# AdeeshKolluru/AdsorbDiff

Measured on AMD Instinct MI355X. Metric: sampled adsorbate sites/sec (50 denoise steps, ~200-atom slabs), higher is better.
Workload: dtype f32 (f16x3-split MFMA, fp32 accumulate; ADF_GEMM=f32 selects exact f32)

## Files before the change

adsorbdiff_amd/csrc/api.hip:

```cpp
#include <stdarg.h>
#include <stdlib.h>
#include <string.h>

#include <new>

#include "common.h"

static thread_local char g_err[512] = "";

void adf_set_error(const char* fmt, ...) {
    va_list ap;
    va_start(ap, fmt);
    vsnprintf(g_err, sizeof(g_err), fmt, ap);
    va_end(ap);
}

extern "C" const char* adf_last_error(void) { return g_err; }
extern "C" const char* adf_version(void) { return "adsorbdiff_hip 0.5.0 (gfx950)"; }

void adf_prof_begin(adf_painn* h, int cat, hipStream_t s) {
    if (!h->prof_on) return;
    if (h->prof_used + 2 > h->prof_ev->size()) {
        for (int i = 0; i < 512; ++i) {
            hipEvent_t e;
// ... 119 lines not shown
        if (st == ADF_OK) st = dev_alloc(&h->w16_scratch, 1);
        if (st == ADF_OK) st = dev_alloc(&h->wfrag_arena, h->w16_bytes);
        {
            const char* ef = getenv("ADF_FUSED_MLP");
            h->fused_mlp = ef ? atoi(ef) : 0;
            if (h->fused_mlp < 0 || h->fused_mlp > 2) h->fused_mlp = 0;
        }
        const char* e = getenv("ADF_GEMM");
        h->gemm_f32 = e && strcmp(e, "f32") == 0;
        const char* el = getenv("ADF_LIFT");
        h->lift_on = !(el && strcmp(el, "0") == 0);
        const char* e2 = getenv("ADF_MSG");
        h->msg_f32 = e2 ? strcmp(e2, "f32") == 0 : h->gemm_f32;
        const char* er = getenv("ADF_ROW_MAXIMA");
        h->rmx = (er && atoi(er) == 0) ? 0 : 1;
    }
    if (st == ADF_OK) st = dev_alloc(&h->kcount, 8);
    if (st == ADF_OK && hipMemset(h->kcount, 0, 8 * sizeof(unsigned long long)) != hipSuccess) st = ADF_EHIP;
    if (st != ADF_OK) { adf_painn_destroy(h); return st; }
    *out = h;
    return ADF_OK;
}

static void inc_free(adf_painn* h) {
    for (int l = 0; l <= ADF_MAX_LAYERS; ++l) {
        if (h->incX[l]) (void)hipFree(h->incX[l]);
        if (h->incV[l]) (void)hipFree(h->incV[l]);
        if (l < ADF_MAX_LAYERS && h->incR[l]) (void)hipFree(h->incR[l]);
        h->incX[l] = h->incV[l] = nullptr;
        if (l < ADF_MAX_LAYERS) h->incR[l] = nullptr;
// ... 295 lines not shown
    if (nbr_src) ADF_HIP_CHECK(hipMemcpyAsync(nbr_src, h->nbr_src, sizeof(int32_t) * N * K, hipMemcpyDeviceToDevice, s));
    if (nbr_shift)
        hipLaunchKernelGGL(adf_export_shift_kernel, dim3((unsigned)((N * K + 255) / 256)), dim3(256), 0, s, h->nbr_shift,
                           nbr_shift, (long long)(N * K), h->last_reps[0], h->last_reps[1], h->last_reps[2]);
    if (edge_src || edge_dst || edge_dist || edge_vec)
        hipLaunchKernelGGL(adf_export_edges_kernel, dim3((unsigned)((N + 3) / 4)), dim3(256), 0, s, h->nptr, h->e_src,
                           h->e_geom, (int)N, edge_src, edge_dst, edge_dist, edge_vec, (long long)edge_capacity);
    ADF_HIP_CHECK(hipGetLastError());
    int32_t e = 0;
    ADF_HIP_CHECK(hipMemcpyAsync(&e, h->nptr + N, sizeof(int32_t), hipMemcpyDeviceToHost, s));
    ADF_HIP_CHECK(hipStreamSynchronize(s));
    if (num_edges) *num_edges = e;
    return ADF_OK;
}

static int32_t zero_pad_rows(adf_painn* h, int N, hipStream_t s) {
    const size_t row = (size_t)5 * h->hp.hidden_channels;
    ADF_HIP_CHECK(hipMemsetAsync(h->rec + (size_t)N * row, 0, sizeof(float) * row, s));
    return ADF_OK;
}

static bool use_fused_mlp(const adf_painn* h, int rows) {
    if (h->hp.hidden_channels != 512 || h->gemm_f32 || h->fused_mlp == 0) return false;
    if (h->fused_mlp == 1) return true;
    return rows >= 2 * 64 * h->num_cus;
}

static int32_t make_records(adf_painn* h, int l, int n, const float* x, const float* vec, bool vec_is_zero, float* rec,
                            const int32_t* row_map, hipStream_t s) {
    const int H = h->hp.hidden_channels;
    const adf_layer_weights& w = h->layer[l];
    if (n <= 0) return ADF_OK;
    adf_prof_begin(h, ADF_PROF_NODE, s);
    const bool lift = h->lift_on && !h->gemm_f32;
    static int emit = -1;
    if (emit < 0) { const char* e = getenv("ADF_LIFT_EMIT"); emit = (e && atoi(e) == 0) ? 0 : 1; }
    const bool em = lift && emit;
    ADF_TRY(adf_nodewise_layernorm(x, w.ln_w, w.ln_b, h->y, n, H, s, em ? h->mag_a : nullptr, h->rows_dev));
    if (use_fused_mlp(h, n) && (em || !lift)) {
        adf_epi ep = {};
        ep.vec_in = vec; ep.rec = rec ? rec : h->rec; ep.H = H; ep.vec_is_zero = vec_is_zero ? 1 : 0;
        ep.row_map = row_map; ep.m_dev = h->rows_dev; ep.lift_y = lift ? 1 : 0;
        ep.rec_rows = row_map ? (long long)h->inc_capN : (long long)n;
        ADF_TRY(adf_launch_mlp16(h->y, nullptr, H, em ? h->mag_a : nullptr, w.xp0_16.frag, &w.xp0_16, w.xp0_b, w.xp2_16.frag, &w.xp2_16, n,
                                 H, 1, &ep, s));
        adf_prof_end(h, s);
        return ADF_OK;
    }
    ADF_TRY(adf_linear(h, h->y, H, w.xp0_w, &w.xp0_16, w.xp0_b, h->cat, H, n, H, H, 1, s, em ? h->mag_a : nullptr,
                       em ? h->mag_b : nullptr));
    if (h->gemm_f32) {
        if (row_map) { adf_set_error("internal: mapped records need the f16x3 path"); return ADF_EINVAL; }
        ADF_TRY(adf_launch_gemm(h->cat, H, w.xp2_w, H, w.xp2_b, h->xh, 3 * H, n, 3 * H, H, 0, s));
        ADF_TRY(adf_pack_records(h, n, h->xh, vec, vec_is_zero, s, rec));
    } else {
        adf_epi ep = {};
        ep.vec_in = vec; ep.rec = rec ? rec : h->rec; ep.H = H; ep.vec_is_zero = vec_is_zero ? 1 : 0;
        ep.row_map = row_map;
        ep.rmag = em ? h->mag_b : nullptr;
        ep.m_dev = h->rows_dev;
        ADF_TRY(adf_launch_gemm16_fused(h->cat, H, &w.xp2_16, n, H, H, 1, &ep, s, lift ? &h->lift : nullptr));
    }
    adf_prof_end(h, s);
    return ADF_OK;
}

static int32_t message_layer(adf_painn* h, int l, int N, const float* x, const float* vec, float* x_out,
                             float* vec_out, bool vec_is_zero, hipStream_t s, const int32_t* tlist = nullptr,
                             int n_targets = 0, float* rec = nullptr, bool records_ready = false) {
    if (!records_ready) ADF_TRY(make_records(h, l, N, x, vec, vec_is_zero, rec, nullptr, s));
    adf_prof_begin(h, ADF_PROF_MESSAGE, s);
    const int items = tlist ? n_targets : N;
// ... 135 lines not shown
    return forward_impl(h, b, out_idx, n_out, f1, f2, stream);
}

static int inc_prepare(adf_painn* h, int N) {
    const int L = h->hp.num_layers, H = h->hp.hidden_channels;
    if (!h->inc_on || !h->moving || h->gemm_f32 || h->msg_f32 || L > ADF_MAX_LAYERS || !h->prev_nptr)
        return 0;
    if (N > h->inc_capN) {
        (void)hipDeviceSynchronize();
        inc_free(h);
        const size_t cap = (size_t)N;
        int32_t st = ADF_OK;
        for (int l = 0; l <= L && st == ADF_OK; ++l) {
            st = dev_alloc(&h->incX[l], cap * H);
            if (st == ADF_OK && l >= 1) st = dev_alloc(&h->incV[l], cap * 3 * H);
            if (st == ADF_OK && l < L) st = dev_alloc(&h->incR[l], (cap + 1) * 5 * H);
        }
        if (st == ADF_OK) st = dev_alloc(&h->inc_c0, cap);
        if (st == ADF_OK) st = dev_alloc(&h->inc_chg, 2 * cap);
        if (st == ADF_OK) st = dev_alloc(&h->inc_pend, cap * L);
        if (st == ADF_OK) st = dev_alloc(&h->inc_need, cap * L);
        if (st == ADF_OK) st = dev_alloc(&h->inc_tf, cap * L);
        if (st == ADF_OK) st = dev_alloc(&h->inc_list, cap * L);
        if (st == ADF_OK) st = dev_alloc(&h->inc_cnt, (size_t)2 * ADF_MAX_LAYERS + 1);
        if (st == ADF_OK) {
            h->inc_tmp_bytes = adf_inc_temp_bytes((int64_t)cap);
            unsigned char* tmp = nullptr;
            st = dev_alloc(&tmp, h->inc_tmp_bytes + 16);
            h->inc_tmp = tmp;
        }
        if (st == ADF_OK && !h->inc_cnt_host &&
// ... 42 lines not shown
    if (peek) return ADF_OK;
    h->inc_ev_live[slot] = false;
    for (int l = 0; l < L; ++l) {
        const bool whole = h->inc_pend_whole[slot][l] != 0;
        h->inc_rows += (unsigned long long)(whole ? N : c[l]);
        h->inc_rows_full += (unsigned long long)N;
        h->inc_edges += (unsigned long long)(whole ? c[2 * L] : c[L + l]);
        if (whole || c[l] > 0) ++h->inc_launches;
    }
    return ADF_OK;
}

static int32_t forward_incremental(adf_painn* h, int N, const int32_t* Z, const int32_t* out_idx, int32_t n_out,
                                   float* f1, float* f2, bool first, int heads, hipStream_t s) {
    const int L = h->hp.num_layers, H = h->hp.hidden_channels;
    const size_t cap = (size_t)h->inc_capN, row = (size_t)5 * H;
    if (out_idx && n_out == 0) return ADF_OK;
    adf_prof_begin(h, ADF_PROF_GRAPH, s);
    if (first) {
        ADF_TRY(adf_nodewise_embed(h, Z, N, h->incX[0], s));
        for (int l = 0; l < L; ++l) ADF_HIP_CHECK(hipMemsetAsync(h->incR[l] + (size_t)N * row, 0, sizeof(float) * row, s));
        ADF_HIP_CHECK(hipMemsetAsync(h->inc_pend, 0, cap * L, s));
    } else {
        ADF_TRY(adf_inc_compare(h, N, s));
    }
    ADF_HIP_CHECK(hipMemsetAsync(h->inc_cnt, 0, sizeof(int32_t) * (2 * ADF_MAX_LAYERS + 1), s));
    if (out_idx) ADF_TRY(adf_inc_need_from_list(h, N, L, out_idx, n_out, s));
    for (int l = 0; l < L; ++l) ADF_TRY(adf_inc_plan_layer(h, l, N, first, out_idx != nullptr, s));
    ADF_HIP_CHECK(hipMemcpyAsync(h->inc_cnt + 2 * L, h->nptr + N, sizeof(int32_t), hipMemcpyDeviceToDevice, s));
    const int slot = h->inc_slot;
    h->inc_slot ^= 1;
    if (h->inc_ev_live[slot]) ADF_TRY(inc_harvest(h, slot, true));
    int32_t* host = h->inc_cnt_host + (size_t)slot * (2 * ADF_MAX_LAYERS + 1);
    ADF_HIP_CHECK(hipMemcpyAsync(host, h->inc_cnt, sizeof(int32_t) * (2 * L + 1), hipMemcpyDeviceToHost, s));
    ADF_HIP_CHECK(hipEventRecord((hipEvent_t)h->inc_ev[slot], s));
    h->inc_ev_live[slot] = true;
// ... 69 lines not shown
    const int heads = head1_only ? 1 : h->hp.num_heads;
    if (heads > h->hp.num_heads) { adf_set_error("the model has no force head"); return ADF_EINVAL; }
    if (!b->atomic_numbers || (heads >= 1 && !f1) || (heads == 2 && !f2)) { adf_set_error("null argument"); return ADF_EINVAL; }
    h->x_last = nullptr;
    hipStream_t s = (hipStream_t)stream;
    const int N = b->num_atoms;
    ADF_TRY(ensure_capacity(h, N, b->num_systems));
    const int inc = inc_prepare(h, N);
    adf_prof_begin(h, ADF_PROF_GRAPH, s);
    ADF_TRY(adf_graph_build_impl(h, b, s));
    adf_prof_end(h, s);
    if (inc) {
        h->inc_serial = h->build_serial;
        return forward_incremental(h, N, b->atomic_numbers, out_idx, n_out, f1, f2, inc == 2, heads, s);
    }
    ADF_TRY(zero_pad_rows(h, N, s));
    ADF_TRY(adf_nodewise_embed(h, b->atomic_numbers, N, h->x, s));
    float* vin = h->vecA;
    float* vout = h->vecB;
    const int L = h->hp.num_layers, H = h->hp.hidden_channels;
    float* rec0 = nullptr;
    bool rec0_ready = false;
    if (h->moving) {
        const size_t row = (size_t)5 * H;
        if ((int64_t)N + 1 > h->rec0_cap) {
            if (h->rec0) { (void)hipFree(h->rec0); h->rec0 = nullptr; }
            h->rec0_cap = 0; h->rec0_valid = false;
            ADF_TRY(dev_alloc(&h->rec0, ((size_t)N + 1) * row));
            h->rec0_cap = (int64_t)N + 1;
        }
        rec0 = h->rec0;
        rec0_ready = h->rec0_valid && h->rec0_N == N;
        if (!rec0_ready) ADF_HIP_CHECK(hipMemsetAsync(rec0 + (size_t)N * row, 0, sizeof(float) * row, s));
        h->rec0_valid = true; h->rec0_N = N;
    }
    if (!out_idx) {
        for (int l = 0; l < L; ++l) {
            if (l == 0) ADF_TRY(message_layer(h, 0, N, h->x, vin, h->x, vout, true, s, nullptr, 0, rec0, rec0_ready));
            else
// ... 287 lines not shown
```

adsorbdiff_amd/csrc/common.h:

```cpp
#pragma once
#include <hip/hip_runtime.h>
#include <stdint.h>
#include <stdio.h>
#include <string>
#include <vector>

#include "../../include/adsorbdiff_hip.h"

#define ADF_GROUP_NODES 32
#define ADF_SLICE_CH 64
#define ADF_MAX_CAND 1024
#define ADF_MAX_K 128
#define ADF_NFLAGS 8
#define ADF_MAX_INDEG 1024
#define ADF_MAX_LAYERS 16

void adf_set_error(const char* fmt, ...);

#define ADF_HIP_CHECK(expr)                                                             \
    do {                                                                                \
        hipError_t _e = (expr);                                                         \
        if (_e != hipSuccess) {                                                         \
            adf_set_error("%s failed: %s (%s:%d)", #expr, hipGetErrorString(_e),        \
                          __FILE__, __LINE__);                                          \
// ... 28 lines not shown
    int H;
    int vec_is_zero;
    const float* A2;
    int K1;
    const int32_t* row_map;
    const float* rmag;
    unsigned int* out_mag;
    const int32_t* m_dev;
    int accumulate;
    int lift_y;
    const float* gate;
    int gate_ld;
    long long rec_rows;
    float* catpart;
    long long part_stride;
};
struct adf_lift {
    float* buf;
    long long cap;
};
struct adf_layer_weights {
    const float *ln_w, *ln_b, *xp0_w, *xp0_b, *xp2_w, *xp2_b, *rbf_w, *rbf_b;
    const float *vp_w, *xv0_w, *xv0_b, *xv2_w, *xv2_b;
    adf_w16 xp0_16, xp2_16, vp_16, xv0_16, xv2_16;
};
struct adf_block_weights {
    const float *vec1_w, *vec2_w, *un0_w, *un0_b, *un2_w, *un2_b;
    adf_w16 vec1_16, vec2_16, un0_16, un2_16;
};

// ... 14 lines not shown
    unsigned char* w16_arena;
    size_t w16_bytes;
    float* w16_scales;
    float* w16_bias_perm;
    unsigned int* w16_scratch;
    unsigned char* wfrag_arena;
    int fused_mlp;
    bool gemm_f32;
    bool msg_f32;
    bool lift_on;
    adf_lift lift;
    float *mag_a, *mag_b;
    float* mag_v3;
    bool mag_v3_valid;
    int rmx;
    float* rmx_part;
    float *xpart, *catpart, *vpart;
    int64_t part_stride;
    const float *part_x, *part_vec;
    int part_n;
    const int32_t* part_dev;
    int dbg_msg_rows, dbg_cat_rows;
    bool dbg_capture;
    float* dbg_mag;
    int dbg_comb_rows;

    int64_t capN, capB, capE;
    int32_t* nbr_cnt;
    int32_t* nbr_src;
    int32_t* nbr_shift;
// ... 138 lines not shown
int32_t adf_inc_need_from_list(adf_painn* h, int N, int L, const int32_t* out_idx, int n_out, hipStream_t s);
int32_t adf_inc_plan_layer(adf_painn* h, int l, int N, bool first, bool have_need, hipStream_t s);
int32_t adf_inc_scatter_rows(const float* src, const int32_t* idx, int n, int width, float* dst, hipStream_t s,
                             const int32_t* n_dev = nullptr);
int32_t adf_inc_gather_rows(const float* src, const int32_t* idx, int n, int width, float* dst, hipStream_t s);
size_t adf_scan_temp_bytes(int64_t n);
int32_t adf_message_impl(adf_painn* h, int layer, int N, const float* x, const float* xh, const float* vec,
                         float* x_out, float* vec_out, bool vec_is_zero, hipStream_t s,
                         const int32_t* tlist = nullptr, int n_targets = 0, const float* rec = nullptr,
                         const int32_t* n_targets_dev = nullptr,
                         float* xpart = nullptr, float* vpart = nullptr, long long part_stride = 0);
int32_t adf_pack_rbf(adf_painn* h, hipStream_t s);
int32_t adf_pack_rbf_layer(adf_painn* h, int l, hipStream_t s);
int32_t adf_pack_records(adf_painn* h, int N, const float* xh, const float* vec, bool vec_is_zero, hipStream_t s,
                         float* rec = nullptr);
int32_t adf_nodewise_embed(adf_painn* h, const int32_t* Z, int N, float* x, hipStream_t s);
int32_t adf_nodewise_layernorm(const float* x, const float* w, const float* b, float* y, int N, int H, hipStream_t s,
                               float* out_mag = nullptr, const int32_t* n_dev = nullptr);
int32_t adf_nodewise_update_prep(const float* vv, const float* x, float* cat, float* dot, int N, int H, hipStream_t s);
int32_t adf_nodewise_update_apply(const float* h3, const float* dot, const float* vv, float* x, float* vec,
                                  float scale, int N, int H, hipStream_t s);
int32_t adf_head_forward(adf_painn* h, int head, int N, const float* x, const float* vec, float* out, hipStream_t s);
int32_t adf_stepper_init(const adf_batch* b, float* pos, const int32_t* tags, const float* noise,
                         hipStream_t s);
int32_t adf_stepper_step(float* sys, const adf_batch* b, float* pos, const int32_t* tags, const int32_t* fixed,
                         const float* f1, const float* f2, const adf_step_coef* coef, const adf_step_coef* coefs_dev,
                         int num_steps, const float* z_tr, const float* z_rot, int32_t early_stop_count,
                         int32_t* state, float* dcom, float* drot, hipStream_t s);
int32_t adf_stepper_tr_step(float* sys, const adf_batch* b, float* pos, const int32_t* tags, const float* f1,
                            const adf_tr_coef* coef, const adf_tr_coef* coefs_dev, int num_steps, const float* z,
// ... 29 lines not shown
```

adsorbdiff_amd/csrc/energy_grad.hip:

```cpp
#include <stdlib.h>
#include <string.h>

#include "message.h"

struct EgW {
    const float* f32;
    adf_w16 w16;
};
enum { EG_XP0 = 0, EG_XP2, EG_VP, EG_XV0, EG_XV2, EG_NW };

struct adf_grad {
    unsigned char* warena;
    float* wscales;
    bool wvalid;
    EgW fw[ADF_MAX_LAYERS][EG_NW];
    EgW bw[ADF_MAX_LAYERS][EG_NW];
    EgW oe_bw;
    float* rbf_wt[ADF_MAX_LAYERS];
    float* act;
    size_t act_floats;
    float4* part;
    int32_t* rev;
    long long ecap;
    int part_slices;
// ... 346 lines not shown
    eg_layout(N, H, L, nullptr, &w);
    if (w.total > g->act_floats || ecap > g->ecap || nslices > g->part_slices) {
        ADF_HIP_CHECK(hipDeviceSynchronize());
        void* old[] = {g->act, g->part, g->rev};
        for (void* p : old)
            if (p) (void)hipFree(p);
        g->act = nullptr; g->part = nullptr; g->rev = nullptr; g->act_floats = 0; g->ecap = 0; g->part_slices = 0;
        const int sl = H / ADF_SLICE_CH;
        ADF_TRY(eg_malloc(reinterpret_cast<void**>(&g->act), w.total * sizeof(float), "activations"));
        ADF_TRY(eg_malloc(reinterpret_cast<void**>(&g->part), (size_t)ecap * sl * sizeof(float4), "per-edge partial gradients"));
        ADF_TRY(eg_malloc(reinterpret_cast<void**>(&g->rev), (size_t)ecap * sizeof(int32_t), "reverse-edge index"));
        g->act_floats = w.total; g->ecap = ecap; g->part_slices = sl;
    }
    eg_layout(N, H, L, g->act, &w);
    const long long pstride = g->ecap;
    const size_t recrow = (size_t)(H / 32) * 160;

    ADF_TRY(adf_nodewise_embed(h, b->atomic_numbers, N, w.layer[0].x, s));
    for (int l = 0; l < L; ++l) {
        const adf_layer_weights& lw = h->layer[l];
        EgLayer& a = w.layer[l];
        const bool vz = l == 0;
        float* xn = l + 1 < L ? w.layer[l + 1].x : w.x_last;
        float* vn = l + 1 < L ? w.layer[l + 1].vec : w.dvecA;
        float *y = w.t1, *c = w.t2, *x1 = w.dx1, *vec1 = w.dvec1, *ua = w.dy;
        ADF_TRY(adf_op_layernorm_fwd(a.x, lw.ln_w, lw.ln_b, y, a.stats, N, H, stream));
        ADF_TRY(eg_lin(h, y, H, g->fw[l][EG_XP0], lw.xp0_b, a.h0, H, N, H, H, s));
        ADF_TRY(adf_op_ssilu_fwd(a.h0, c, (int64_t)N * H, stream));
        ADF_TRY(eg_lin(h, c, H, g->fw[l][EG_XP2], lw.xp2_b, a.xh, 3 * H, N, 3 * H, H, s));
        ADF_HIP_CHECK(hipMemsetAsync(h->rec + (size_t)N * recrow, 0, sizeof(float) * recrow, s));
        ADF_TRY(adf_pack_records(h, N, a.xh, a.vec, vz, s));
        {
            const bool prof = h->prof_on;
            h->prof_on = false;
            const int32_t st = adf_message_impl(h, l, N, a.x, a.xh, a.vec, x1, vec1, vz, s);
            h->prof_on = prof;
            ADF_TRY(st);
        }
        ADF_TRY(eg_lin(h, vec1, H, g->fw[l][EG_VP], nullptr, a.vv, 2 * H, 3ll * N, 2 * H, H, s));
        ADF_TRY(adf_op_copy_rows(x1, H, a.cat, 2 * H, N, H, 0, stream));
        ADF_TRY(adf_op_vdot_fwd(a.vv, a.dot, a.cat + H, 2 * H, N, H, 1e-8f, stream));
        ADF_TRY(eg_lin(h, a.cat, 2 * H, g->fw[l][EG_XV0], lw.xv0_b, a.u0, H, N, H, 2 * H, s));
        ADF_TRY(adf_op_ssilu_fwd(a.u0, ua, (int64_t)N * H, stream));
        ADF_TRY(eg_lin(h, ua, H, g->fw[l][EG_XV2], lw.xv2_b, a.a, 3 * H, N, 3 * H, H, s));
// ... 55 lines not shown
```

adsorbdiff_amd/csrc/gemm16.hip:

```cpp
#include <stdlib.h>

#include "common.h"

typedef float f32x16 __attribute__((ext_vector_type(16)));
typedef _Float16 half8 __attribute__((ext_vector_type(8)));
typedef _Float16 half4 __attribute__((ext_vector_type(4)));

#ifndef EPI_ABL
#define EPI_ABL 0
#endif
#ifndef EPI2_POLICY
#define EPI2_POLICY 0
#endif
#ifndef G16_ABL
#define G16_ABL 0
#endif
#ifndef G16_WDEEP
#define G16_WDEEP 1
#endif
#define HK 32
#define TLD3 96
#define TLD2 64
#define HLD 40

// ... 475 lines not shown
                        const int n = min(m0 + wm + 32 * i + it * 8 + (lane >> 3), M - 1);
                        const float* vr = ep.vec_in + (size_t)n * 3 * H + c;
                        v0[it] = *reinterpret_cast<const float4*>(vr);
                        v1[it] = *reinterpret_cast<const float4*>(vr + H);
                        v2[it] = *reinterpret_cast<const float4*>(vr + 2 * H);
                    }
                }
#pragma unroll
                for (int it = 0; it < 4; ++it) {
                    const int lr = it * 8 + (lane >> 3);
                    const int n = m0 + wm + 32 * i + lr;
                    const float4 p0 = *reinterpret_cast<const float4*>(T + lr * TLD3 + 4 * c4);
                    const float4 p1 = *reinterpret_cast<const float4*>(T + lr * TLD3 + 32 + 4 * c4);
                    const float4 p2 = *reinterpret_cast<const float4*>(T + lr * TLD3 + 64 + 4 * c4);
                    if ((EPI_ABL & 8) && n >= 0) { if (ep.H < 0) ep.rec[0] = p0.x + p1.x + p2.x + v0[it].x + v1[it].y + v2[it].z; }
                    else if (n < M) {
                        float* rec = ep.rec + ((size_t)(ep.row_map ? ep.row_map[n] : n) * (H / 32) + g) * 160;
                        float4* ra_ = reinterpret_cast<float4*>(rec + 16 * c4);
                        if (!ep.vec_is_zero) {
                            ra_[0] = make_float4(v0[it].x * p1.x, v1[it].x * p1.x, v2[it].x * p1.x, p0.x);
                            ra_[1] = make_float4(v0[it].y * p1.y, v1[it].y * p1.y, v2[it].y * p1.y, p0.y);
                            ra_[2] = make_float4(v0[it].z * p1.z, v1[it].z * p1.z, v2[it].z * p1.z, p0.z);
                            ra_[3] = make_float4(v0[it].w * p1.w, v1[it].w * p1.w, v2[it].w * p1.w, p0.w);
                        } else {
                            ra_[0] = make_float4(0.f, 0.f, 0.f, p0.x);
                            ra_[1] = make_float4(0.f, 0.f, 0.f, p0.y);
                            ra_[2] = make_float4(0.f, 0.f, 0.f, p0.z);
                            ra_[3] = make_float4(0.f, 0.f, 0.f, p0.w);
                        }
                        *reinterpret_cast<float4*>(rec + 128 + 4 * c4) = p2;
                    }
// ... 322 lines not shown
```

adsorbdiff_amd/csrc/message.h:

```cpp
#pragma once
#include "common.h"

typedef float f32x16 __attribute__((ext_vector_type(16)));
typedef _Float16 half8 __attribute__((ext_vector_type(8)));

#define MSG_THREADS 512
#define MSG_WAVES 8
#define MSG_COLS 192
#define MSG_LDK 136

struct MsgParams {
    const float* rec;
    const float* vec;
    const float* x;
    float* x_out;
    float* vec_out;
    const int32_t* tlist;
    int items;
    const int32_t* items_dev;
    const int32_t* nptr;
    const int32_t* e_src;
    const float4* e_geom;
    const float* wpack;
    const _Float16* wpack16;
    const float* bpack;
    const float* inv_scale;
    const float* mu;
    int N, H, R, G, nslices;
    float inv_cutoff, coeff, sarg, env_a, env_b, env_c;
    float dmu2, dmusq, cstep;
    int env_pi;
    unsigned long long* kcount;
    float* xpart;
    float* vpart;
    long long part_stride;
};
int32_t adf_pack_grad_records(adf_painn* h, const float* gx1, const float* gv1, float* dx, hipStream_t s);
```

adsorbdiff_amd/csrc/message.hip:

```cpp
#include <stdlib.h>
#include <string.h>

#include "message.h"

#ifndef MSG_ABL
#define MSG_ABL 0
#endif
#ifndef MSG_SKIP
#define MSG_SKIP 1
#endif
#ifndef MSG_EXP_NOXC
#define MSG_EXP_NOXC 0
#endif

__device__ __forceinline__ float wave_min(float v) {
#pragma unroll
    for (int o = 32; o > 0; o >>= 1) v = fminf(v, __shfl_xor(v, o));
    return v;
}
__device__ __forceinline__ float wave_max(float v) {
#pragma unroll
    for (int o = 32; o > 0; o >>= 1) v = fmaxf(v, __shfl_xor(v, o));
    return v;
}
// ... 50 lines not shown
            const int n4 = p.R * MSG_COLS / 4;
            for (int i = tid; i < n4; i += FWD_THREADS) dst[i] = src[i];
        }
        if (!F16 && tid < MSG_COLS) Bl[tid] = p.bpack[slice * MSG_COLS + tid];
        if (tid < 144) Mu[tid] = (tid < p.R ? p.mu[tid] : 2.0f) * (F16 ? p.sarg : 1.0f);
        if (tid == 0) *Ctr = 0;
    }
    __syncthreads();
    float* meta_w = Meta + wave * 32 * 8;
    const float inv_sqrt3 = 0.57735026918962576f;
    const float inv_sqrt2 = 0.70710678118654752f;
    const float out_scale = F16 ? *p.inv_scale * (1.0f / 256.0f) : 1.0f;
    const float inv_sqrt_h = out_scale / sqrtf((float)H);
    const float umax_scale = (float)(p.R - 1);
    const float coeff2 = p.coeff * 1.44269504088896341f;
    const unsigned int row_bytes = (unsigned int)p.nslices * 1280u;
    const char* recS = reinterpret_cast<const char*>(p.rec) + (size_t)slice * 1280;
    const unsigned int qA = (unsigned int)q * 16u;
    const unsigned int qP = 512u + (unsigned int)q * 4u;

    unsigned int ksteps = 0;

    typedef const __attribute__((address_space(4))) int32_t* cint_ptr;
    const cint_ptr nptr_c = (cint_ptr)p.nptr;
    const cint_ptr tlist_c = (cint_ptr)p.tlist;
    auto fetch_target = [&](int& n_out, int& o_out) -> bool {
        while (true) {
            int t = 0;
            if (lane == 0) t = atomicAdd(Ctr, 1);
            t = __builtin_amdgcn_readfirstlane(t);
            const int g = worker + (t >> 5) * nworkers;
            if (g >= ngroups) return false;
            const int e = g * ADF_GROUP_NODES + (t & 31);
            if (e < items) { o_out = e; n_out = p.tlist ? tlist_c[e] : e; return true; }
// ... 69 lines not shown
                klo = max(0, (int)floorf(umin) - 7) & ~1;
                khi = min(p.R, ((int)ceilf(umax) + 8 + 1) & ~1);
            }
            klo = __builtin_amdgcn_readfirstlane(klo);
            khi = __builtin_amdgcn_readfirstlane(khi);
            ksteps += (khi - klo) * (VZ && F16 ? 4 : 6);

#define ROW_OF(r) ((r & 3) + 8 * (r >> 2) + 4 * hi)
#define DECL(r)                                                                                 \
    const float* m##r = meta_w + ROW_OF(r) * 8;                                                 \
    float4 ga0##r, ga1##r;                                      \
    float gz0##r, gz1##r;
#define GATHER(r)                                                                               \
    {                                                                                           \
    const unsigned int o##r = __float_as_uint(m##r[0]);                                         \
    if (MSG_EXP_NOXC) { gz0##r = 1.0f; gz1##r = 2.0f; } else {                                 \
    gz0##r = *reinterpret_cast<const float*>(recS + (size_t)(o##r + qP));                       \
    gz1##r = *reinterpret_cast<const float*>(recS + (size_t)(o##r + qP) + 640); }               \
    if (MSG_EXP_NOXC == 2) { ga0##r = make_float4(1.f, 2.f, 3.f, 4.f); ga1##r = ga0##r; }      \
    else if (!VZ) {                                                                             \
        ga0##r = *reinterpret_cast<const float4*>(recS + (size_t)(o##r + qA));                  \
        ga1##r = *reinterpret_cast<const float4*>(recS + (size_t)(o##r + qA) + 640);            \
    } else {                                                                                    \
        ga0##r = make_float4(0.f, 0.f, 0.f, *reinterpret_cast<const float*>(recS + (size_t)(o##r + qA) + 12)); \
        ga1##r = make_float4(0.f, 0.f, 0.f, *reinterpret_cast<const float*>(recS + (size_t)(o##r + qA) + 652)); \
    }                                                                                           \
    }
#define CONSUME(r)                                                                              \
    {                                                                                           \
        const float ux = m##r[1], uy = m##r[2], uz = m##r[3];                                   \
        const float t3 = gz0##r * acc[4][r];                                                    \
        sx0 += ga0##r.w * acc[0][r];                                                            \
        if (!VZ) { sa0 += ga0##r.x * acc[2][r]; sb0 += ga0##r.y * acc[2][r]; sc0 += ga0##r.z * acc[2][r]; } \
        ra0 += t3 * ux; rb0 += t3 * uy; rc0 += t3 * uz;                                         \
        const float u3 = gz1##r * acc[5][r];                                                    \
        sx1 += ga1##r.w * acc[1][r];                                                            \
        if (!VZ) { sa1 += ga1##r.x * acc[3][r]; sb1 += ga1##r.y * acc[3][r]; sc1 += ga1##r.z * acc[3][r]; } \
        ra1 += u3 * ux; rb1 += u3 * uy; rc1 += u3 * uz;                                         \
    }
            DECL(0) DECL(1) DECL(2) DECL(3) DECL(4) DECL(5) DECL(6) DECL(7)
// ... 238 lines not shown
        const size_t base = (size_t)slice * 2 * MSG_COLS * R;
        wpack16[base + (size_t)col * R + k] = h;
        wpack16[base + (size_t)(MSG_COLS + col) * R + k] = (_Float16)(v - (float)h);
        if (k == 0) {
            const float bv = b[part * H + ch] * scale;
            const _Float16 bh = (_Float16)bv;
            _Float16* o = reinterpret_cast<_Float16*>(bpack16 + slice * MSG_COLS + col);
            o[0] = bh; o[1] = (_Float16)(bv - (float)bh);
        }
    }
}

__global__ void adf_absmax_kernel(const float* __restrict__ w, long long n, unsigned int* out_bits);

__global__ void adf_pack_records_kernel(const float* __restrict__ xh, const float* __restrict__ vec,
                                        float* __restrict__ rec, int N, int H, int vec_is_zero) {
    const int ng = H / 32;
    const long long total = (long long)N * ng * 32;
    for (long long t = (long long)blockIdx.x * blockDim.x + threadIdx.x; t < total;
         t += (long long)gridDim.x * blockDim.x) {
        const int qq = (int)(t & 31);
        const int g = (int)((t >> 5) % ng);
        const long long n = t / (32LL * ng);
        const int c = 32 * g + qq;
        const float* xr = xh + (size_t)n * 3 * H;
        const float xa = xr[c], xb = xr[H + c], xc = xr[2 * H + c];
        float* out = rec + ((size_t)n * ng + g) * 160;
        if (!vec_is_zero) {
            const float* vr = vec + (size_t)n * 3 * H;
            reinterpret_cast<float4*>(out)[qq] = make_float4(vr[c] * xb, vr[H + c] * xb, vr[2 * H + c] * xb, xa);
        } else {
            reinterpret_cast<float4*>(out)[qq] = make_float4(0.f, 0.f, 0.f, xa);
        }
        out[128 + qq] = xc;
    }
}

int32_t adf_pack_records(adf_painn* h, int N, const float* xh, const float* vec, bool vec_is_zero, hipStream_t s,
                         float* rec) {
    const int H = h->hp.hidden_channels;
    long long blocks = ((long long)N * H + 255) / 256;
    if (blocks > 256 * 16) blocks = 256 * 16;
    hipLaunchKernelGGL(adf_pack_records_kernel, dim3((unsigned)blocks), dim3(256), 0, s, xh, vec, rec ? rec : h->rec, N, H,
                       vec_is_zero ? 1 : 0);
    ADF_HIP_CHECK(hipGetLastError());
    return ADF_OK;
}

static size_t msg_lds_bytes(int R, bool f16) {
    const size_t w = f16 ? (size_t)2 * MSG_COLS * MSG_LDK * 2 : sizeof(float) * (size_t)R * MSG_COLS;
    return w + sizeof(float) * (MSG_COLS + 144 + FWD_WAVES * 32 * 8) + 16;
}

int32_t adf_pack_rbf_layer(adf_painn* h, int l, hipStream_t s) {
    const int H = h->hp.hidden_channels, R = h->hp.num_rbf;
    const size_t per_layer = (size_t)(H / ADF_SLICE_CH) * R * MSG_COLS;
    const size_t per_layer_b = (size_t)(H / ADF_SLICE_CH) * MSG_COLS;
    hipLaunchKernelGGL(adf_pack_rbf_kernel, dim3(256), dim3(256), 0, s, h->layer[l].rbf_w, h->layer[l].rbf_b,
                       h->rbf_pack + l * per_layer, h->rbf_bias_pack + l * per_layer_b, H, R);
// ... 55 lines not shown
    p.N = N; p.H = H; p.R = R;
    p.tlist = tlist; p.items = tlist ? n_targets : N; p.items_dev = tlist ? n_targets_dev : nullptr;
    if (p.items <= 0) return ADF_OK;
    p.G = (p.items + ADF_GROUP_NODES - 1) / ADF_GROUP_NODES;
    p.inv_cutoff = 1.0f / h->hp.cutoff;
    const double step = 1.0 / (R - 1);
    p.coeff = (float)(-0.5 / (step * step));
    p.sarg = (float)sqrt(0.5 / (step * step) * 1.4426950408889634);
    const double pe = (double)h->hp.envelope_exponent;
    p.env_pi = h->hp.envelope_exponent;
    p.env_a = (float)(-(pe + 1) * (pe + 2) / 2);
    p.env_b = (float)(pe * (pe + 2));
    p.env_c = (float)(-pe * (pe + 1) / 2);
    p.kcount = h->prof_on ? h->kcount : nullptr;
    p.xpart = xpart; p.vpart = xpart ? vpart : nullptr; p.part_stride = part_stride;
    int workers = h->num_cus / p.nslices;
    if (workers < 1) workers = 1;
    if (workers > p.G) workers = p.G;
    dim3 grid((unsigned)(workers * p.nslices));
#define LAUNCH_MSG(F16_, VZ_, UNI_)                                                                        \
    hipLaunchKernelGGL((adf_message_kernel<F16_, VZ_, UNI_>), grid, dim3(FWD_THREADS), msg_lds_bytes(R, F16_), s, p)
    {
        const double d = sqrt(0.5 / (step * step) * 1.4426950408889634) * step;
        p.dmu2 = (float)(2.0 * d); p.dmusq = (float)(d * d); p.cstep = (float)exp2(-2.0 * d * d);
    }
    if (f16 && h->rbf_uniform) { if (vec_is_zero) LAUNCH_MSG(true, true, true); else LAUNCH_MSG(true, false, true); }
    else if (f16) { if (vec_is_zero) LAUNCH_MSG(true, true, false); else LAUNCH_MSG(true, false, false); }
    else { if (vec_is_zero) LAUNCH_MSG(false, true, false); else LAUNCH_MSG(false, false, false); }
#undef LAUNCH_MSG
    ADF_HIP_CHECK(hipGetLastError());
// ... 3 lines not shown
```

adsorbdiff_amd/csrc/mlp16.hip:

```cpp
#include "common.h"

typedef float f32x16 __attribute__((ext_vector_type(16)));
typedef _Float16 half8 __attribute__((ext_vector_type(8)));
typedef _Float16 half4 __attribute__((ext_vector_type(4)));

#ifndef ML_ABL
#define ML_ABL 0
#endif
#ifndef ML_VAR
#define ML_VAR 0
#endif
#ifndef ML_PROF
#define ML_PROF 0
#endif
#if ML_PROF
#define ML_STAMP(k_) do { if (lane == 0 && (wave & 3) == 0) { const unsigned long long t_ = wall_clock64(); \
        atomicAdd(reinterpret_cast<unsigned long long*>(ml_prof) + (wave >> 2) * 8 + (k_), t_ - ml_t); ml_t = t_; } } while (0)
#else
#define ML_STAMP(k_) do { } while (0)
#endif
#define ML_H 512
#define ML_TM 64
#define ML_YLD 1040
#define ML_PLANE (ML_TM * ML_YLD)
// ... 355 lines not shown
                    const float sc = isc2 * rinvY[8 * band + l8];
                    T[l8 * 96 + q] = acc[i][0][r] * sc + bb0;
                    T[l8 * 96 + 32 + q] = acc[i][1][r] * sc + bb1;
                    T[l8 * 96 + 64 + q] = acc[i][2][r] * sc + bb2;
                }
                __builtin_amdgcn_fence(__ATOMIC_RELEASE, "wavefront");
                __builtin_amdgcn_wave_barrier();
                const float4 p0 = *reinterpret_cast<const float4*>(T + lr * 96 + 4 * c4);
                const float4 p1 = *reinterpret_cast<const float4*>(T + lr * 96 + 32 + 4 * c4);
                const float4 p2 = *reinterpret_cast<const float4*>(T + lr * 96 + 64 + 4 * c4);
                const float4 e0 = eo[bb][0], e1 = eo[bb][1], e2 = eo[bb][2];
                if (ML_ABL & 1) {
                    const float sk = p0.x + p1.y + p2.z + e0.x + e1.y + e2.z;
                    asm volatile("" ::"v"(sk));
                } else if constexpr (EPI == 1) {
                    if (n_raw < M) {
                        const unsigned int ro = ((unsigned int)(ep.row_map ? ep.row_map[n] : n) * (unsigned int)(H / 32) + (unsigned int)g) * 640u;
                        float* rec = reinterpret_cast<float*>(rec_b + ro);
                        float4* ra_ = reinterpret_cast<float4*>(rec + 16 * c4);
                        if (!ep.vec_is_zero) {
                            ra_[0] = make_float4(e0.x * p1.x, e1.x * p1.x, e2.x * p1.x, p0.x);
                            ra_[1] = make_float4(e0.y * p1.y, e1.y * p1.y, e2.y * p1.y, p0.y);
                            ra_[2] = make_float4(e0.z * p1.z, e1.z * p1.z, e2.z * p1.z, p0.z);
                            ra_[3] = make_float4(e0.w * p1.w, e1.w * p1.w, e2.w * p1.w, p0.w);
                        } else {
                            ra_[0] = make_float4(0.f, 0.f, 0.f, p0.x);
                            ra_[1] = make_float4(0.f, 0.f, 0.f, p0.y);
                            ra_[2] = make_float4(0.f, 0.f, 0.f, p0.z);
                            ra_[3] = make_float4(0.f, 0.f, 0.f, p0.w);
                        }
                        *reinterpret_cast<float4*>(rec + 128 + 4 * c4) = p2;
// ... 58 lines not shown
```

adsorbdiff_amd/csrc/train.hip:

```cpp
#include <stdlib.h>
#include <string.h>

#include "common.h"

typedef float f32x16 __attribute__((ext_vector_type(16)));

#define TR_CHECK_LAUNCH() ADF_HIP_CHECK(hipGetLastError())

static inline unsigned tr_grid(long long total, int per_block = 256) {
    long long b = (total + per_block - 1) / per_block;
    if (b > 256 * 16) b = 256 * 16;
    if (b < 1) b = 1;
    return (unsigned)b;
}

__device__ __forceinline__ float tr_wsum(float v) {
#pragma unroll
    for (int o = 32; o > 0; o >>= 1) v += __shfl_xor(v, o);
    return v;
}

__device__ __forceinline__ float tr_ssilu(float x) { return x / (1.0f + expf(-x)) * 1.6666666666666667f; }
__device__ __forceinline__ float tr_dssilu(float x) {
    const float s = 1.0f / (1.0f + expf(-x));
// ... 704 lines not shown
                                      float* x1, float* vec1, int32_t vec_is_zero, void* stream) {
    if (!h || h->lastN <= 0) { adf_set_error("message_fwd: no graph"); return ADF_EINVAL; }
    hipLaunchKernelGGL(tr_msg_fwd_kernel, dim3((unsigned)h->lastN), dim3(256), 0, (hipStream_t)stream, h->nptr, h->e_src,
                       h->e_geom, xh, vec, rbfh, x, x1, vec1, h->hp.hidden_channels, vec_is_zero);
    TR_CHECK_LAUNCH();
    return ADF_OK;
}
extern "C" int32_t adf_op_message_fwd_fused(adf_painn_t h, int32_t layer, const float* xh, const float* vec, const float* x,
                                            float* x1, float* vec1, int32_t vec_is_zero, void* stream) {
    if (!h || h->lastN <= 0 || !h->weights_set || layer < 0 || layer >= h->hp.num_layers || !xh || !x || !x1 || !vec1 ||
        (!vec && !vec_is_zero)) {
        adf_set_error("message_fwd_fused: bad argument or no graph");
        return ADF_EINVAL;
    }
    hipStream_t s = (hipStream_t)stream;
    const int N = (int)h->lastN, H = h->hp.hidden_channels;
    const size_t row = (size_t)(H / 32) * 160;
    ADF_TRY(adf_pack_rbf_layer(h, layer, s));
    ADF_HIP_CHECK(hipMemsetAsync(h->rec + (size_t)N * row, 0, sizeof(float) * row, s));
    ADF_TRY(adf_pack_records(h, N, xh, vec, vec_is_zero != 0, s));
    return adf_message_impl(h, layer, N, x, xh, vec, x1, vec1, vec_is_zero != 0, s);
}
extern "C" int32_t adf_op_message_bwd(adf_painn_t h, const float* xh, const float* vec, const float* rbfh, const float* gx1,
                                      const float* gv1, float* dxh, float* drbfh, float* dvec, float* dx,
                                      int32_t vec_is_zero, void* stream) {
    if (!h || h->lastN <= 0) { adf_set_error("message_bwd: no graph"); return ADF_EINVAL; }
    hipLaunchKernelGGL(tr_msg_bwd_kernel, dim3((unsigned)h->lastN), dim3(256), 0, (hipStream_t)stream, h->nptr, h->e_src,
                       h->e_geom, xh, vec, rbfh, gx1, gv1, dxh, drbfh, dvec, dx, h->hp.hidden_channels, vec_is_zero);
    TR_CHECK_LAUNCH();
    return ADF_OK;
}

// ... 300 lines not shown
```

Measured before the change: 254.3.

## Compact layer-0 message records to two channels when input vectors are zero

```diff
diff --git a/adsorbdiff_amd/csrc/api.hip b/adsorbdiff_amd/csrc/api.hip
--- a/adsorbdiff_amd/csrc/api.hip
+++ b/adsorbdiff_amd/csrc/api.hip
@@ -157,6 +157,8 @@
         h->msg_f32 = e2 ? strcmp(e2, "f32") == 0 : h->gemm_f32;
         const char* er = getenv("ADF_ROW_MAXIMA");
         h->rmx = (er && atoi(er) == 0) ? 0 : 1;
+        const char* ec = getenv("ADF_REC0_COMPACT");
+        h->rec0c = (ec && atoi(ec) == 0) ? 0 : 1;
     }
     if (st == ADF_OK) st = dev_alloc(&h->kcount, 8);
     if (st == ADF_OK && hipMemset(h->kcount, 0, 8 * sizeof(unsigned long long)) != hipSuccess) st = ADF_EHIP;
@@ -482,9 +484,13 @@
     return ADF_OK;
 }
 
-static int32_t zero_pad_rows(adf_painn* h, int N, hipStream_t s) {
-    const size_t row = (size_t)5 * h->hp.hidden_channels;
+static int32_t zero_pad_rows(adf_painn* h, int N, hipStream_t s, bool layer0_in_rec = false) {
+    const size_t row = adf_rec_row_floats(h, false);
     ADF_HIP_CHECK(hipMemsetAsync(h->rec + (size_t)N * row, 0, sizeof(float) * row, s));
+    if (layer0_in_rec && adf_rec_compact(h, true)) {
+        const size_t row0 = adf_rec_row_floats(h, true);
+        ADF_HIP_CHECK(hipMemsetAsync(h->rec + (size_t)N * row0, 0, sizeof(float) * row0, s));
+    }
     return ADF_OK;
 }
 
@@ -508,6 +514,7 @@
     if (use_fused_mlp(h, n) && (em || !lift)) {
         adf_epi ep = {};
         ep.vec_in = vec; ep.rec = rec ? rec : h->rec; ep.H = H; ep.vec_is_zero = vec_is_zero ? 1 : 0;
+        ep.rec_compact = adf_rec_compact(h, vec_is_zero) ? 1 : 0;
         ep.row_map = row_map; ep.m_dev = h->rows_dev; ep.lift_y = lift ? 1 : 0;
         ep.rec_rows = row_map ? (long long)h->inc_capN : (long long)n;
         ADF_TRY(adf_launch_mlp16(h->y, nullptr, H, em ? h->mag_a : nullptr, w.xp0_16.frag, &w.xp0_16, w.xp0_b, w.xp2_16.frag, &w.xp2_16, n,
@@ -524,6 +531,7 @@
     } else {
         adf_epi ep = {};
         ep.vec_in = vec; ep.rec = rec ? rec : h->rec; ep.H = H; ep.vec_is_zero = vec_is_zero ? 1 : 0;
+        ep.rec_compact = adf_rec_compact(h, vec_is_zero) ? 1 : 0;
         ep.row_map = row_map;
         ep.rmag = em ? h->mag_b : nullptr;
         ep.m_dev = h->rows_dev;
@@ -689,7 +697,7 @@
         for (int l = 0; l <= L && st == ADF_OK; ++l) {
             st = dev_alloc(&h->incX[l], cap * H);
             if (st == ADF_OK && l >= 1) st = dev_alloc(&h->incV[l], cap * 3 * H);
-            if (st == ADF_OK && l < L) st = dev_alloc(&h->incR[l], (cap + 1) * 5 * H);
+            if (st == ADF_OK && l < L) st = dev_alloc(&h->incR[l], (cap + 1) * adf_rec_row_floats(h, l == 0));
         }
         if (st == ADF_OK) st = dev_alloc(&h->inc_c0, cap);
         if (st == ADF_OK) st = dev_alloc(&h->inc_chg, 2 * cap);
@@ -762,12 +770,15 @@
 static int32_t forward_incremental(adf_painn* h, int N, const int32_t* Z, const int32_t* out_idx, int32_t n_out,
                                    float* f1, float* f2, bool first, int heads, hipStream_t s) {
     const int L = h->hp.num_layers, H = h->hp.hidden_channels;
-    const size_t cap = (size_t)h->inc_capN, row = (size_t)5 * H;
+    const size_t cap = (size_t)h->inc_capN;
     if (out_idx && n_out == 0) return ADF_OK;
     adf_prof_begin(h, ADF_PROF_GRAPH, s);
     if (first) {
         ADF_TRY(adf_nodewise_embed(h, Z, N, h->incX[0], s));
-        for (int l = 0; l < L; ++l) ADF_HIP_CHECK(hipMemsetAsync(h->incR[l] + (size_t)N * row, 0, sizeof(float) * row, s));
+        for (int l = 0; l < L; ++l) {
+            const size_t row = adf_rec_row_floats(h, l == 0);
+            ADF_HIP_CHECK(hipMemsetAsync(h->incR[l] + (size_t)N * row, 0, sizeof(float) * row, s));
+        }
         ADF_HIP_CHECK(hipMemsetAsync(h->inc_pend, 0, cap * L, s));
     } else {
         ADF_TRY(adf_inc_compare(h, N, s));
@@ -867,7 +878,7 @@
         h->inc_serial = h->build_serial;
         return forward_incremental(h, N, b->atomic_numbers, out_idx, n_out, f1, f2, inc == 2, heads, s);
     }
-    ADF_TRY(zero_pad_rows(h, N, s));
+    ADF_TRY(zero_pad_rows(h, N, s, !h->moving));
     ADF_TRY(adf_nodewise_embed(h, b->atomic_numbers, N, h->x, s));
     float* vin = h->vecA;
     float* vout = h->vecB;
@@ -875,7 +886,7 @@
     float* rec0 = nullptr;
     bool rec0_ready = false;
     if (h->moving) {
-        const size_t row = (size_t)5 * H;
+        const size_t row = adf_rec_row_floats(h, true);
         if ((int64_t)N + 1 > h->rec0_cap) {
             if (h->rec0) { (void)hipFree(h->rec0); h->rec0 = nullptr; }
             h->rec0_cap = 0; h->rec0_valid = false;
diff --git a/adsorbdiff_amd/csrc/common.h b/adsorbdiff_amd/csrc/common.h
--- a/adsorbdiff_amd/csrc/common.h
+++ b/adsorbdiff_amd/csrc/common.h
@@ -66,6 +66,7 @@
     long long rec_rows;
     float* catpart;
     long long part_stride;
+    int rec_compact;
 };
 struct adf_lift {
     float* buf;
@@ -110,6 +111,7 @@
     float* mag_v3;
     bool mag_v3_valid;
     int rmx;
+    int rec0c;
     float* rmx_part;
     float *xpart, *catpart, *vpart;
     int64_t part_stride;
@@ -278,6 +280,10 @@
 int32_t adf_pack_rbf_layer(adf_painn* h, int l, hipStream_t s);
 int32_t adf_pack_records(adf_painn* h, int N, const float* xh, const float* vec, bool vec_is_zero, hipStream_t s,
                          float* rec = nullptr);
+static inline bool adf_rec_compact(const adf_painn* h, bool vec_is_zero) { return vec_is_zero && h->rec0c != 0; }
+static inline size_t adf_rec_row_floats(const adf_painn* h, bool vec_is_zero) {
+    return (size_t)(adf_rec_compact(h, vec_is_zero) ? 2 : 5) * (size_t)h->hp.hidden_channels;
+}
 int32_t adf_nodewise_embed(adf_painn* h, const int32_t* Z, int N, float* x, hipStream_t s);
 int32_t adf_nodewise_layernorm(const float* x, const float* w, const float* b, float* y, int N, int H, hipStream_t s,
                                float* out_mag = nullptr, const int32_t* n_dev = nullptr);
diff --git a/adsorbdiff_amd/csrc/energy_grad.hip b/adsorbdiff_amd/csrc/energy_grad.hip
--- a/adsorbdiff_amd/csrc/energy_grad.hip
+++ b/adsorbdiff_amd/csrc/energy_grad.hip
@@ -384,7 +384,6 @@
     }
     eg_layout(N, H, L, g->act, &w);
     const long long pstride = g->ecap;
-    const size_t recrow = (size_t)(H / 32) * 160;
 
     ADF_TRY(adf_nodewise_embed(h, b->atomic_numbers, N, w.layer[0].x, s));
     for (int l = 0; l < L; ++l) {
@@ -398,6 +397,7 @@
         ADF_TRY(eg_lin(h, y, H, g->fw[l][EG_XP0], lw.xp0_b, a.h0, H, N, H, H, s));
         ADF_TRY(adf_op_ssilu_fwd(a.h0, c, (int64_t)N * H, stream));
         ADF_TRY(eg_lin(h, c, H, g->fw[l][EG_XP2], lw.xp2_b, a.xh, 3 * H, N, 3 * H, H, s));
+        const size_t recrow = adf_rec_row_floats(h, vz);
         ADF_HIP_CHECK(hipMemsetAsync(h->rec + (size_t)N * recrow, 0, sizeof(float) * recrow, s));
         ADF_TRY(adf_pack_records(h, N, a.xh, a.vec, vz, s));
         {
diff --git a/adsorbdiff_amd/csrc/gemm16.hip b/adsorbdiff_amd/csrc/gemm16.hip
--- a/adsorbdiff_amd/csrc/gemm16.hip
+++ b/adsorbdiff_amd/csrc/gemm16.hip
@@ -513,7 +513,11 @@
                     const float4 p1 = *reinterpret_cast<const float4*>(T + lr * TLD3 + 32 + 4 * c4);
                     const float4 p2 = *reinterpret_cast<const float4*>(T + lr * TLD3 + 64 + 4 * c4);
                     if ((EPI_ABL & 8) && n >= 0) { if (ep.H < 0) ep.rec[0] = p0.x + p1.x + p2.x + v0[it].x + v1[it].y + v2[it].z; }
-                    else if (n < M) {
+                    else if (n < M && ep.rec_compact) {
+                        float* rec = ep.rec + ((size_t)(ep.row_map ? ep.row_map[n] : n) * (H / 32) + g) * 64;
+                        *reinterpret_cast<float4*>(rec + 4 * c4) = p0;
+                        *reinterpret_cast<float4*>(rec + 32 + 4 * c4) = p2;
+                    } else if (n < M) {
                         float* rec = ep.rec + ((size_t)(ep.row_map ? ep.row_map[n] : n) * (H / 32) + g) * 160;
                         float4* ra_ = reinterpret_cast<float4*>(rec + 16 * c4);
                         if (!ep.vec_is_zero) {
diff --git a/adsorbdiff_amd/csrc/message.h b/adsorbdiff_amd/csrc/message.h
--- a/adsorbdiff_amd/csrc/message.h
+++ b/adsorbdiff_amd/csrc/message.h
@@ -34,5 +34,6 @@
     float* xpart;
     float* vpart;
     long long part_stride;
+    int rec_compact;
 };
 int32_t adf_pack_grad_records(adf_painn* h, const float* gx1, const float* gv1, float* dx, hipStream_t s);
diff --git a/adsorbdiff_amd/csrc/message.hip b/adsorbdiff_amd/csrc/message.hip
--- a/adsorbdiff_amd/csrc/message.hip
+++ b/adsorbdiff_amd/csrc/message.hip
@@ -88,10 +88,15 @@
     const float inv_sqrt_h = out_scale / sqrtf((float)H);
     const float umax_scale = (float)(p.R - 1);
     const float coeff2 = p.coeff * 1.44269504088896341f;
-    const unsigned int row_bytes = (unsigned int)p.nslices * 1280u;
-    const char* recS = reinterpret_cast<const char*>(p.rec) + (size_t)slice * 1280;
+    const bool cmp = VZ && p.rec_compact;
+    const unsigned int half_bytes = cmp ? 256u : 640u;
+    const unsigned int row_bytes = VZ ? (unsigned int)p.nslices * (2u * half_bytes) : (unsigned int)p.nslices * 1280u;
+    const char* recS = reinterpret_cast<const char*>(p.rec) + (VZ ? (size_t)slice * (2u * half_bytes) : (size_t)slice * 1280);
     const unsigned int qA = (unsigned int)q * 16u;
     const unsigned int qP = 512u + (unsigned int)q * 4u;
+    const char* recS1 = recS + half_bytes;
+    const unsigned int qXa = cmp ? (unsigned int)q * 4u : qA + 12u;
+    const unsigned int qXc = cmp ? 128u + (unsigned int)q * 4u : qP;
 
     unsigned int ksteps = 0;
 
@@ -191,16 +196,18 @@
 #define GATHER(r)                                                                               \
     {                                                                                           \
     const unsigned int o##r = __float_as_uint(m##r[0]);                                         \
-    if (MSG_EXP_NOXC) { gz0##r = 1.0f; gz1##r = 2.0f; } else {                                 \
+    if (MSG_EXP_NOXC) { gz0##r = 1.0f; gz1##r = 2.0f; } else if (!VZ) {                        \
     gz0##r = *reinterpret_cast<const float*>(recS + (size_t)(o##r + qP));                       \
-    gz1##r = *reinterpret_cast<const float*>(recS + (size_t)(o##r + qP) + 640); }               \
+    gz1##r = *reinterpret_cast<const float*>(recS + (size_t)(o##r + qP) + 640); } else {        \
+    gz0##r = *reinterpret_cast<const float*>(recS + (size_t)(o##r + qXc));                      \
+    gz1##r = *reinterpret_cast<const float*>(recS1 + (size_t)(o##r + qXc)); }                   \
     if (MSG_EXP_NOXC == 2) { ga0##r = make_float4(1.f, 2.f, 3.f, 4.f); ga1##r = ga0##r; }      \
     else if (!VZ) {                                                                             \
         ga0##r = *reinterpret_cast<const float4*>(recS + (size_t)(o##r + qA));                  \
         ga1##r = *reinterpret_cast<const float4*>(recS + (size_t)(o##r + qA) + 640);            \
     } else {                                                                                    \
-        ga0##r = make_float4(0.f, 0.f, 0.f, *reinterpret_cast<const float*>(recS + (size_t)(o##r + qA) + 12)); \
-        ga1##r = make_float4(0.f, 0.f, 0.f, *reinterpret_cast<const float*>(recS + (size_t)(o##r + qA) + 652)); \
+        ga0##r = make_float4(0.f, 0.f, 0.f, *reinterpret_cast<const float*>(recS + (size_t)(o##r + qXa)));  \
+        ga1##r = make_float4(0.f, 0.f, 0.f, *reinterpret_cast<const float*>(recS1 + (size_t)(o##r + qXa))); \
     }                                                                                           \
     }
 #define CONSUME(r)                                                                              \
@@ -469,7 +476,7 @@
 __global__ void adf_absmax_kernel(const float* __restrict__ w, long long n, unsigned int* out_bits);
 
 __global__ void adf_pack_records_kernel(const float* __restrict__ xh, const float* __restrict__ vec,
-                                        float* __restrict__ rec, int N, int H, int vec_is_zero) {
+                                        float* __restrict__ rec, int N, int H, int vec_is_zero, int compact) {
     const int ng = H / 32;
     const long long total = (long long)N * ng * 32;
     for (long long t = (long long)blockIdx.x * blockDim.x + threadIdx.x; t < total;
@@ -480,6 +487,12 @@
         const int c = 32 * g + qq;
         const float* xr = xh + (size_t)n * 3 * H;
         const float xa = xr[c], xb = xr[H + c], xc = xr[2 * H + c];
+        if (compact) {
+            float* outc = rec + ((size_t)n * ng + g) * 64;
+            outc[qq] = xa;
+            outc[32 + qq] = xc;
+            continue;
+        }
         float* out = rec + ((size_t)n * ng + g) * 160;
         if (!vec_is_zero) {
             const float* vr = vec + (size_t)n * 3 * H;
@@ -497,7 +510,7 @@
     long long blocks = ((long long)N * H + 255) / 256;
     if (blocks > 256 * 16) blocks = 256 * 16;
     hipLaunchKernelGGL(adf_pack_records_kernel, dim3((unsigned)blocks), dim3(256), 0, s, xh, vec, rec ? rec : h->rec, N, H,
-                       vec_is_zero ? 1 : 0);
+                       vec_is_zero ? 1 : 0, adf_rec_compact(h, vec_is_zero) ? 1 : 0);
     ADF_HIP_CHECK(hipGetLastError());
     return ADF_OK;
 }
@@ -583,6 +596,7 @@
     p.env_c = (float)(-pe * (pe + 1) / 2);
     p.kcount = h->prof_on ? h->kcount : nullptr;
     p.xpart = xpart; p.vpart = xpart ? vpart : nullptr; p.part_stride = part_stride;
+    p.rec_compact = adf_rec_compact(h, vec_is_zero) ? 1 : 0;
     int workers = h->num_cus / p.nslices;
     if (workers < 1) workers = 1;
     if (workers > p.G) workers = p.G;
diff --git a/adsorbdiff_amd/csrc/mlp16.hip b/adsorbdiff_amd/csrc/mlp16.hip
--- a/adsorbdiff_amd/csrc/mlp16.hip
+++ b/adsorbdiff_amd/csrc/mlp16.hip
@@ -393,7 +393,12 @@
                     const float sk = p0.x + p1.y + p2.z + e0.x + e1.y + e2.z;
                     asm volatile("" ::"v"(sk));
                 } else if constexpr (EPI == 1) {
-                    if (n_raw < M) {
+                    if (n_raw < M && ep.rec_compact) {
+                        const unsigned int ro = ((unsigned int)(ep.row_map ? ep.row_map[n] : n) * (unsigned int)(H / 32) + (unsigned int)g) * 256u;
+                        float* rec = reinterpret_cast<float*>(rec_b + ro);
+                        *reinterpret_cast<float4*>(rec + 4 * c4) = p0;
+                        *reinterpret_cast<float4*>(rec + 32 + 4 * c4) = p2;
+                    } else if (n_raw < M) {
                         const unsigned int ro = ((unsigned int)(ep.row_map ? ep.row_map[n] : n) * (unsigned int)(H / 32) + (unsigned int)g) * 640u;
                         float* rec = reinterpret_cast<float*>(rec_b + ro);
                         float4* ra_ = reinterpret_cast<float4*>(rec + 16 * c4);
diff --git a/adsorbdiff_amd/csrc/train.hip b/adsorbdiff_amd/csrc/train.hip
--- a/adsorbdiff_amd/csrc/train.hip
+++ b/adsorbdiff_amd/csrc/train.hip
@@ -742,8 +742,8 @@
         return ADF_EINVAL;
     }
     hipStream_t s = (hipStream_t)stream;
-    const int N = (int)h->lastN, H = h->hp.hidden_channels;
-    const size_t row = (size_t)(H / 32) * 160;
+    const int N = (int)h->lastN;
+    const size_t row = adf_rec_row_floats(h, vec_is_zero != 0);
     ADF_TRY(adf_pack_rbf_layer(h, layer, s));
     ADF_HIP_CHECK(hipMemsetAsync(h->rec + (size_t)N * row, 0, sizeof(float) * row, s));
     ADF_TRY(adf_pack_records(h, N, xh, vec, vec_is_zero != 0, s));
```

Result: no change. 256.3, median of 6 (+0.8%).
